# timghill/GladsGP

Hardware: NVIDIA B200
Metric: mcmc_steps_per_s (higher is better)
Workload: dtype f64

## Files before the change

gladsgp_b200/csrc/ggp_mcmc.cu:

```cuda
#include "ggp_chol.cuh"
#include "../../include/gladsgp_b200.h"

namespace ggp {

enum { PRIOR_UNIFORM = 0, PRIOR_GAMMA = 1, PRIOR_BETA = 2, PRIOR_NORMAL = 3 };
enum { PROP_UNIFORM = 0, PROP_BETARHO = 1, PROP_PROPMH = 2 };

__device__ inline double elem_log_prior(int kind, double a, double b, double x)
{
    switch (kind) {
        case PRIOR_GAMMA: return (a - 1.0) * log(x) - b * x;
        case PRIOR_BETA: {
            double rho = exp(-x / 4.0);
            if (rho > 0.999) rho = 0.999;
            return (a - 1.0) * log(rho) + (b - 1.0) * log(1.0 - rho);
        }
        case PRIOR_NORMAL: {
            double z = (x - a) / b;
            return -0.5 * (z * z);
        }
        default: return 0.0;
    }
}

struct Plan {
    double* cand;
    double* lacorr;
    double* logu;
    int* valid;
};

__device__ inline void plan_chain(const ggp_mcmc_args& a, const Plan& pl, int t, int c)
{
    const int P = a.d * a.pu + 2 * a.pu + 1;
    const double* th = a.theta + (size_t)c * P;
    const double* step = a.step + (size_t)t * a.step_stride_t + (size_t)c * a.step_stride_c;
    long long pos = a.upos ? a.upos[c] : 0;
    const double* us = a.uniforms ? a.uniforms + (size_t)c * a.n_uniform : nullptr;
    for (int s = 0; s < P; ++s) {
        const size_t o = (size_t)c * P + s;
        double cand, lac = 0.0, lu = 0.0;
        int valid;
        if (a.fixed[s] == 2) {
            pl.cand[o] = th[s]; pl.lacorr[o] = 0.0; pl.logu[o] = 0.0; pl.valid[o] = 0;
            continue;
        }
        if (a.replay) {
            const size_t ro = ((size_t)t * a.n_chains + c) * P + s;
            cand = a.r_cand[ro];
            lac = a.r_logacorr[ro];
            lu = a.r_logu[ro];
            valid = a.r_valid[ro] && !a.fixed[s];
        } else {
            const double x = th[s];
            const double st = step[s];
            const double u = us[pos++];
            double acorr = 1.0;
            int kind = a.prop_kind[s];
            if (kind == PROP_PROPMH && !a.do_propMH) kind = PROP_UNIFORM;
            if (kind == PROP_UNIFORM) {
                cand = __dadd_rn(x, __dmul_rn(st, __dadd_rn(-0.5, u)));
            } else if (kind == PROP_BETARHO) {
                const double rho = __dadd_rn(exp(-x / 4.0), __dmul_rn(st, __dadd_rn(-0.5, u)));
                cand = (rho <= 0.0) ? INFINITY : -4.0 * log(rho);
            } else {
                const double w = fmax(1.0, x / 3.0);
                cand = __dadd_rn(x, __dmul_rn(w, __dadd_rn(-1.0, __dmul_rn(2.0, u))));
                const double w1 = fmax(1.0, cand / 3.0);
                acorr = (x > cand + w1) ? 0.0 : w / w1;
            }
            valid = !a.fixed[s] && (acorr > 0.0) && (cand >= a.lo[s]) && (cand <= a.hi[s]);
            if (valid) {
                lu = log(us[pos++]);
                lac = log(acorr);
            }
        }
        pl.cand[o] = cand;
        pl.lacorr[o] = lac;
        pl.logu[o] = lu;
        pl.valid[o] = valid;
    }
    if (a.upos) a.upos[c] = pos;
}

__global__ void plan_kernel(ggp_mcmc_args a, Plan pl, int t)
{
    const int c = blockIdx.x * blockDim.x + threadIdx.x;
    if (c < a.n_chains) plan_chain(a, pl, t, c);
}

__device__ __forceinline__ const double* chain_w(const ggp_mcmc_args& a, int c, int j)
{
    return a.W + ((size_t)(a.per_chain_data ? c : 0) * a.pu + j) * a.m;
}
__device__ __forceinline__ double chain_lamsim(const ggp_mcmc_args& a, int c, int j)
{
    return a.lamsim[(size_t)(a.per_chain_data ? c : 0) * a.pu + j];
}
__device__ __forceinline__ size_t chain_prior_off(const ggp_mcmc_args& a, int c)
{
    return a.per_chain_data ? (size_t)c * ((size_t)a.d * a.pu + 2 * a.pu + 1) : 0;
}

__device__ inline void gather_block_params(const ggp_mcmc_args& a, const double* th, int c, int j, int site, double cand,
                                           double* beta_sm, double& lamz, double& diag_add)
{
    const int d = a.d, pu = a.pu, P = d * pu + 2 * pu + 1;
    if (threadIdx.x < d) {
        const int s = j * d + threadIdx.x;
        beta_sm[threadIdx.x] = (s == site) ? cand : th[s];
    }
    const int sz = d * pu + j, ss = d * pu + pu + j, so = P - 1;
    lamz = (sz == site) ? cand : th[sz];
    const double lamws = (ss == site) ? cand : th[ss];
    const double lamwos = (so == site) ? cand : th[so];
    diag_add = 1.0 / (chain_lamsim(a, c, j) * lamwos) + 1.0 / lamws;
}

#ifndef GGP_EVAL_INLINE
#define GGP_EVAL_INLINE 0
#endif
#if GGP_EVAL_INLINE
#define GGP_EVAL_ATTR __forceinline__
#else
#define GGP_EVAL_ATTR __noinline__
#endif
static __device__ GGP_EVAL_ATTR double eval_la_call(unsigned char* smem_raw, const double* __restrict__ X, int m, int Mp, int d,
                                                    const double* beta, double lamz, double diag_add,
                                                    const double* __restrict__ w, double* __restrict__ Lp, int rot)
{
    LaSmem sm = carve_la_smem(smem_raw, Mp, d);
    return eval_block_loglik_la(sm, X, m, Mp, d, beta, lamz, diag_add, w, Lp, nullptr, nullptr, rot);
}

template <bool CL, bool LA, int RA>
static __device__ __forceinline__ double eval_dispatch(unsigned char* smem_raw, const double* __restrict__ X, int m, int Mp, int d,
                                                       const double* beta, double lamz, double diag_add,
                                                       const double* __restrict__ w, double* __restrict__ Lp, int rot = 0)
{
    if constexpr (LA) {
        return eval_la_call(smem_raw, X, m, Mp, d, beta, lamz, diag_add, w, Lp, rot);
    } else {
        EvalSmem sm = carve_eval_smem(smem_raw, Mp, d);
        return eval_block_loglik<CL, RA>(sm, X, m, Mp, d, beta, lamz, diag_add, w, Lp, nullptr, nullptr);
    }
}

__device__ inline void finalize_chain(const ggp_mcmc_args& a, const Plan& pl, const double* __restrict__ sig_cand, int t, int c)
{
    const int d = a.d, pu = a.pu, P = d * pu + 2 * pu + 1;
    double* th = a.theta + (size_t)c * P;
    double* sig = a.sigwl + (size_t)c * pu;
    const int s = P - 1;
    const size_t o = (size_t)c * P + s;
    int acc = 0;
    if (pl.valid[o]) {
        double sn = 0.0, so = 0.0;
        for (int j = 0; j < pu; ++j) {
            sn += sig_cand[(size_t)c * pu + j];
            so += sig[j];
        }
        const double cand = pl.cand[o];
        const size_t po = chain_prior_off(a, c) + s;
        const double dprior = elem_log_prior(a.prior_kind[s], a.prior_a[po], a.prior_b[po], cand) -
                              elem_log_prior(a.prior_kind[s], a.prior_a[po], a.prior_b[po], th[s]);
        acc = pl.logu[o] < ((sn - so) + dprior) + pl.lacorr[o];
        if (acc) {
            th[s] = cand;
            for (int j = 0; j < pu; ++j) sig[j] = sig_cand[(size_t)c * pu + j];
        }
    }
    if (a.accepted) a.accepted[((size_t)t * a.n_chains + c) * P + s] = (unsigned char)acc;
    if (a.lp_draws) {
        double ll = 0.0;
        for (int j = 0; j < pu; ++j) ll += sig[j];
        double lpr = 0.0;
        const int bounds[5] = {0, d * pu, d * pu + pu, d * pu + 2 * pu, P};
        for (int blk = 0; blk < 4; ++blk) {
            if (a.fixed[bounds[blk]] == 2) continue;
            double sblk = 0.0;
            for (int e = bounds[blk]; e < bounds[blk + 1]; ++e)
                sblk += elem_log_prior(a.prior_kind[e], a.prior_a[chain_prior_off(a, c) + e], a.prior_b[chain_prior_off(a, c) + e], th[e]);
            lpr += sblk;
        }
        a.lp_draws[(size_t)t * a.n_chains + c] = ll + lpr;
    }
    if (a.draws) {
        double* dr = a.draws + ((size_t)t * a.n_chains + c) * P;
        for (int e = 0; e < P; ++e) dr[e] = th[e];
    }
}

template <bool CL, bool LA = false, int RA = GGP_RA>
__global__ void __launch_bounds__(NT, CL ? GGP_CL_CTAS_PER_SM : GGP_CTAS_PER_SM)
sweep_kernel(ggp_mcmc_args a, Plan pl, double* __restrict__ Lws, long long l_stride, double* __restrict__ sig_cand,
             unsigned* __restrict__ arrive, int t)
{
    extern __shared__ __align__(16) unsigned char smem_raw[];
    const int Mp = round_up32(a.m);
    __shared__ double beta_sm[64];
    const int j = a.pc_begin + (CL ? blockIdx.x / cluster_nctarank() : blockIdx.x), c = blockIdx.y;
    const bool lead = (threadIdx.x == 0) && (!CL || cluster_ctarank() == 0);
    const int d = a.d, pu = a.pu, P = d * pu + 2 * pu + 1;
    double* th = a.theta + (size_t)c * P;
    double* sig = a.sigwl + (size_t)c * pu;
    double* Lp = Lws + ((size_t)c * pu + j) * l_stride;
    const double* wj = chain_w(a, c, j);
    unsigned char* accd = a.accepted ? a.accepted + ((size_t)t * a.n_chains + c) * P : nullptr;
    const int rot = LA ? cta_role_rotation() : 0;
    const bool shard = a.pc_count > 0;
    double* xrow = shard ? a.xchg + ((size_t)j * a.n_chains + c) * (2 * d + 6) : nullptr;
    if (shard && lead) {
        xrow[d + 3] = sig[j];
        for (int e = 0; e < d + 2; ++e) xrow[d + 4 + e] = 0.0;
    }

    for (int sl = 0; sl < d + 3; ++sl) {
        const bool wos = (sl == d + 2);
        const int s = wos ? P - 1 : ((sl < d) ? j * d + sl : (sl == d ? d * pu + j : d * pu + pu + j));
        const size_t o = (size_t)c * P + s;
        const int valid = pl.valid[o];
        if (!valid) {
            if (lead && accd && !wos) accd[s] = 0;
            continue;
        }
        const double cand = pl.cand[o];
        double lamz, diag_add;
        __syncthreads();
        gather_block_params(a, th, c, j, s, cand, beta_sm, lamz, diag_add);
        __syncthreads();
        const double ll_new = eval_dispatch<CL, LA, RA>(smem_raw, a.X, a.m, Mp, d, beta_sm, lamz, diag_add, wj, Lp, rot);
        if (lead) {
            if (a.eval_count) atomicAdd(a.eval_count + (wos ? 1 : 0), 1ULL);
            if (wos) {
                sig_cand[(size_t)c * pu + j] = ll_new;
            } else {
                const double ll_old = sig[j];
                const double xold = th[s];
                const size_t po = chain_prior_off(a, c) + s;
                const double dprior = elem_log_prior(a.prior_kind[s], a.prior_a[po], a.prior_b[po], cand) -
                                      elem_log_prior(a.prior_kind[s], a.prior_a[po], a.prior_b[po], xold);
                const bool acc = pl.logu[o] < ((ll_new - ll_old) + dprior) + pl.lacorr[o];
                if (acc) {
                    th[s] = cand;
                    sig[j] = ll_new;
                }
                if (accd) accd[s] = acc ? 1 : 0;
                if (shard) xrow[d + 4 + sl] = acc ? 1.0 : 0.0;
            }
        }
        if (CL) cluster_sync_all();
        else __syncthreads();
    }
    if (lead && shard) {
        for (int e = 0; e < d; ++e) xrow[e] = th[j * d + e];
        xrow[d] = th[d * pu + j];
        xrow[d + 1] = th[d * pu + pu + j];
        xrow[d + 2] = sig[j];
        if (pl.valid[(size_t)c * P + (P - 1)]) xrow[d + 3] = sig_cand[(size_t)c * pu + j];
    } else if (lead) {
        __threadfence();
        const unsigned prev = atomicAdd(&arrive[c], 1u);
        if (prev == (unsigned)pu - 1u) {
            arrive[c] = 0u;
            __threadfence();
            finalize_chain(a, pl, sig_cand, t, c);
            if (t + 1 < a.n_steps) plan_chain(a, pl, t + 1, c);
        }
    }
}

constexpr int SPEC_LANES = 3;
constexpr int SPEC_MAXEV = 72;

__device__ __forceinline__ unsigned ld_acquire_u32(const unsigned* p)
{
    unsigned v;
    asm volatile("ld.acquire.gpu.global.u32 %0, [%1];" : "=r"(v) : "l"(p) : "memory");
    return v;
}

__device__ inline void gather_spec(const ggp_mcmc_args& a, const double* st, double lamwos_cur, int c, int j,
                                   int ea, double ca, int eb, double cb, double* beta_sm, double& lamz, double& diag_add)
{
    const int d = a.d;
    if (threadIdx.x < d) {
        const int e = threadIdx.x;
        beta_sm[e] = (e == ea) ? ca : ((e == eb) ? cb : st[e]);
    }
    lamz = (ea == d) ? ca : ((eb == d) ? cb : st[d]);
    const double lamws = (ea == d + 1) ? ca : ((eb == d + 1) ? cb : st[d + 1]);
    const double lamwos = (ea == d + 2) ? ca : ((eb == d + 2) ? cb : lamwos_cur);
    diag_add = 1.0 / (chain_lamsim(a, c, j) * lamwos) + 1.0 / lamws;
}

struct SpecWs {
    double* res;
    unsigned* cnt;
    double* state;
    double* Lws;
};

template <int RA>
__global__ void __launch_bounds__(NT, GGP_CL_CTAS_PER_SM)
sweep_spec_kernel(ggp_mcmc_args a, Plan pl, SpecWs sw, long long l_stride, double* __restrict__ sig_cand,
                  unsigned* __restrict__ arrive, int t, unsigned round_base)
{
    extern __shared__ __align__(16) unsigned char smem_raw[];
    __shared__ double beta_sm[64];
    __shared__ int ev_sm[SPEC_MAXEV];
    __shared__ int nev_sm;
    const int Mp = round_up32(a.m);
    const int G = (int)cluster_nctarank();
    const int cl = blockIdx.x / G;
    const int jl = cl / SPEC_LANES, lane_id = cl - jl * SPEC_LANES, c = blockIdx.y;
    const int j = a.pc_begin + jl;
    const bool lead = (threadIdx.x == 0) && (cluster_ctarank() == 0);
    const bool shard = a.pc_count > 0;
    const int d = a.d, pu = a.pu, P = d * pu + 2 * pu + 1;
    const int E = d + 3;
    double* th = a.theta + (size_t)c * P;
    double* st = sw.state + (((size_t)c * pu + j) * SPEC_LANES + lane_id) * (d + 3);
    double* Lp = sw.Lws + (((size_t)c * pu + j) * SPEC_LANES + lane_id) * l_stride;
    double* res = sw.res + ((size_t)c * pu + j) * 8;
    unsigned* cnt = sw.cnt + (size_t)c * pu + j;
    const double* wj = chain_w(a, c, j);
    unsigned char* accd = a.accepted ? a.accepted + ((size_t)t * a.n_chains + c) * P : nullptr;
    const double lamwos_cur = th[P - 1];
    double* xrow = shard ? a.xchg + ((size_t)j * a.n_chains + c) * (2 * d + 6) : nullptr;
    if (shard && lead && lane_id == 0) {
        xrow[d + 3] = a.sigwl[(size_t)c * pu + j];
        for (int e = 0; e < d + 2; ++e) xrow[d + 4 + e] = 0.0;
    }
    auto site_of = [&](int e) { return e < d ? j * d + e : (e == d ? d * pu + j : (e == d + 1 ? d * pu + pu + j : P - 1)); };

    if (threadIdx.x == 0) {
        int n = 0;
        for (int e = 0; e < E; ++e) {
            if (pl.valid[(size_t)c * P + site_of(e)]) ev_sm[n++] = e;
            else if (lead && accd && lane_id == 0 && e < d + 2) accd[site_of(e)] = 0;
        }
        nev_sm = n;
        if (cluster_ctarank() == 0) {
            for (int e = 0; e < d; ++e) st[e] = th[j * d + e];
            st[d] = th[d * pu + j];
            st[d + 1] = th[d * pu + pu + j];
            st[d + 2] = a.sigwl[(size_t)c * pu + j];
        }
    }
    cluster_sync_all();
    const int nev = nev_sm;
    const int nrounds = (nev + 1) >> 1;

    for (int r = 0; r < nrounds; ++r) {
        const int e0 = ev_sm[2 * r];
        const int e1 = (2 * r + 1 < nev) ? ev_sm[2 * r + 1] : -1;
        const size_t o0 = (size_t)c * P + site_of(e0);
        const size_t o1 = (e1 >= 0) ? (size_t)c * P + site_of(e1) : 0;
        const double c0 = pl.cand[o0];
        const double c1 = (e1 >= 0) ? pl.cand[o1] : 0.0;
        const bool work = (lane_id == 0) || (e1 >= 0);
        double ll = 0.0;
        if (work) {
            double lamz, diag_add;
            __syncthreads();
            if (lane_id == 0) gather_spec(a, st, lamwos_cur, c, j, e0, c0, -1, 0.0, beta_sm, lamz, diag_add);
            else if (lane_id == 1) gather_spec(a, st, lamwos_cur, c, j, e0, c0, e1, c1, beta_sm, lamz, diag_add);
            else gather_spec(a, st, lamwos_cur, c, j, e1, c1, -1, 0.0, beta_sm, lamz, diag_add);
            __syncthreads();
            ll = eval_dispatch<true, false, RA>(smem_raw, a.X, a.m, Mp, d, beta_sm, lamz, diag_add, wj, Lp, 0);
        }
        if (lead) {
            if (work && a.eval_count) atomicAdd(a.eval_count, 1ULL);
            double* slot = res + (r & 1) * 4;
            slot[lane_id] = ll;
            __threadfence();
            atomicAdd(cnt, 1u);
            const unsigned target = (round_base + (unsigned)r + 1u) * SPEC_LANES;
            const long long t0 = clock64();
            bool ok = true;
            while ((int)(ld_acquire_u32(cnt) - target) < 0) {
                if (clock64() - t0 > (1LL << 33)) { ok = false; break; }
            }
            const double l0 = __ldcg(slot + 0), l1a = __ldcg(slot + 1), l1r = __ldcg(slot + 2);
            if (!ok && a.lp_draws) a.lp_draws[(size_t)t * a.n_chains + c] = NAN;
            bool acc0 = false;
            if (e0 == d + 2) {
                if (lane_id == 0) sig_cand[(size_t)c * pu + j] = l0;
            } else {
                const int s0 = site_of(e0);
                const size_t po = chain_prior_off(a, c) + s0;
                const double dprior = elem_log_prior(a.prior_kind[s0], a.prior_a[po], a.prior_b[po], c0) -
                                      elem_log_prior(a.prior_kind[s0], a.prior_a[po], a.prior_b[po], st[e0]);
                acc0 = pl.logu[o0] < ((l0 - st[d + 2]) + dprior) + pl.lacorr[o0];
                if (acc0) { st[e0] = c0; st[d + 2] = l0; }
                if (accd && lane_id == 0) accd[s0] = acc0 ? 1 : 0;
                if (shard && lane_id == 0) xrow[d + 4 + e0] = acc0 ? 1.0 : 0.0;
            }
            if (e1 >= 0) {
                const double l1 = acc0 ? l1a : l1r;
                if (e1 == d + 2) {
                    if (lane_id == 0) sig_cand[(size_t)c * pu + j] = l1;
                } else {
                    const int s1 = site_of(e1);
                    const size_t po = chain_prior_off(a, c) + s1;
                    const double dprior = elem_log_prior(a.prior_kind[s1], a.prior_a[po], a.prior_b[po], c1) -
                                          elem_log_prior(a.prior_kind[s1], a.prior_a[po], a.prior_b[po], st[e1]);
                    const bool acc1 = pl.logu[o1] < ((l1 - st[d + 2]) + dprior) + pl.lacorr[o1];
                    if (acc1) { st[e1] = c1; st[d + 2] = l1; }
                    if (accd && lane_id == 0) accd[s1] = acc1 ? 1 : 0;
                    if (shard && lane_id == 0) xrow[d + 4 + e1] = acc1 ? 1.0 : 0.0;
                }
            }
        }
        cluster_sync_all();
    }
    if (lead) {
        const int rcap = (E + 1) >> 1;
        if (nrounds < rcap) atomicAdd(cnt, (unsigned)(rcap - nrounds));
        if (lane_id == 0 && shard) {
            for (int e = 0; e < d + 3; ++e) xrow[e] = st[e];
            if (pl.valid[(size_t)c * P + (P - 1)]) xrow[d + 3] = sig_cand[(size_t)c * pu + j];
        } else if (lane_id == 0) {
            for (int e = 0; e < d; ++e) th[j * d + e] = st[e];
            th[d * pu + j] = st[d];
            th[d * pu + pu + j] = st[d + 1];
            a.sigwl[(size_t)c * pu + j] = st[d + 2];
            __threadfence();
            const unsigned prev = atomicAdd(&arrive[c], 1u);
            if (prev == (unsigned)pu - 1u) {
                arrive[c] = 0u;
                __threadfence();
                finalize_chain(a, pl, sig_cand, t, c);
                if (t + 1 < a.n_steps) plan_chain(a, pl, t + 1, c);
            }
        }
    }
}

template <bool CL, bool LA = false, int RA = GGP_RA>
__global__ void __launch_bounds__(NT, CL ? GGP_CL_CTAS_PER_SM : GGP_CTAS_PER_SM)
eval_all_kernel(ggp_mcmc_args a, Plan pl, double* __restrict__ Lws, long long l_stride,
                double* __restrict__ sig_cand, int mode)
{
    extern __shared__ __align__(16) unsigned char smem_raw[];
    const int Mp = round_up32(a.m);
    __shared__ double beta_sm[64];
    const int j = CL ? blockIdx.x / cluster_nctarank() : blockIdx.x, c = blockIdx.y;
    const int d = a.d, pu = a.pu, P = d * pu + 2 * pu + 1;
    const double* th = a.theta + (size_t)c * P;
    double* Lp = Lws + ((size_t)c * pu + j) * l_stride;
    int site = -1;
    double cand = 0.0;
    if (mode == 1) {
        const size_t o = (size_t)c * P + (P - 1);
        if (!pl.valid[o]) return;
        site = P - 1;
        cand = pl.cand[o];
    }
    double lamz, diag_add;
    const int rot = LA ? cta_role_rotation() : 0;
    gather_block_params(a, th, c, j, site, cand, beta_sm, lamz, diag_add);
    __syncthreads();
    const double ll = eval_dispatch<CL, LA, RA>(smem_raw, a.X, a.m, Mp, d, beta_sm, lamz, diag_add, chain_w(a, c, j), Lp, rot);
    if (threadIdx.x == 0 && (!CL || cluster_ctarank() == 0)) {
        if (mode == 0) a.sigwl[(size_t)c * pu + j] = ll;
        else sig_cand[(size_t)c * pu + j] = ll;
        if (a.eval_count) atomicAdd(a.eval_count + 1, 1ULL);
    }
}

__global__ void close_kernel(ggp_mcmc_args a, Plan pl, double* __restrict__ sig_cand, int t, int plan_next)
{
    const int c = blockIdx.x * blockDim.x + threadIdx.x;
    if (c >= a.n_chains) return;
    const int d = a.d, pu = a.pu, P = d * pu + 2 * pu + 1;
    double* th = a.theta + (size_t)c * P;
    double* sig = a.sigwl + (size_t)c * pu;
    unsigned char* accd = a.accepted ? a.accepted + ((size_t)t * a.n_chains + c) * P : nullptr;
    for (int j = 0; j < pu; ++j) {
        const double* row = a.xchg + ((size_t)j * a.n_chains + c) * (2 * d + 6);
        for (int e = 0; e < d; ++e) th[j * d + e] = row[e];
        th[d * pu + j] = row[d];
        th[d * pu + pu + j] = row[d + 1];
        sig[j] = row[d + 2];
        sig_cand[(size_t)c * pu + j] = row[d + 3];
        if (accd) {
            for (int e = 0; e < d; ++e) accd[j * d + e] = (unsigned char)(row[d + 4 + e] != 0.0);
            accd[d * pu + j] = (unsigned char)(row[d + 4 + d] != 0.0);
            accd[d * pu + pu + j] = (unsigned char)(row[d + 4 + d + 1] != 0.0);
        }
    }
    finalize_chain(a, pl, sig_cand, t, c);
    if (plan_next) plan_chain(a, pl, t + 1, c);
}

static size_t align256(size_t x) { return (x + 255) & ~(size_t)255; }

static int spec_cluster_size(int pu, int n_chains, int Mp, int d)
{
    if (const char* e = getenv("GGP_SPEC")) { if (atoi(e) == 0) return 0; }
    if (d + 3 > SPEC_MAXEV) return 0;
    const int g_plain = choose_cluster((long long)pu * n_chains, Mp);
    if (g_plain <= 1) return 0;
    const int g_spec = choose_cluster((long long)SPEC_LANES * pu * n_chains, Mp);
    return (g_spec >= 2 && 2 * g_spec > g_plain) ? g_spec : 0;
}

struct McmcWs {
    double* Lws; Plan pl; double* sig_cand; unsigned* arrive; SpecWs spec;
};
long long workspace_bytes_impl(int m, int d, int pu, int n_chains, bool with_spec);

static McmcWs carve_ws(const ggp_mcmc_args& a)
{
    const int Mp = round_up32(a.m);
    const size_t P = (size_t)a.d * a.pu + 2 * a.pu + 1;
    McmcWs w;
    unsigned char* p = reinterpret_cast<unsigned char*>(a.workspace);
    w.Lws = reinterpret_cast<double*>(p);
    p += align256((size_t)a.n_chains * a.pu * packed_doubles(Mp) * sizeof(double));
    w.pl.cand = reinterpret_cast<double*>(p);   p += align256((size_t)a.n_chains * P * sizeof(double));
    w.pl.lacorr = reinterpret_cast<double*>(p); p += align256((size_t)a.n_chains * P * sizeof(double));
    w.pl.logu = reinterpret_cast<double*>(p);   p += align256((size_t)a.n_chains * P * sizeof(double));
    w.pl.valid = reinterpret_cast<int*>(p);     p += align256((size_t)a.n_chains * P * sizeof(int));
    w.sig_cand = reinterpret_cast<double*>(p);  p += align256((size_t)a.n_chains * a.pu * sizeof(double));
    w.arrive = reinterpret_cast<unsigned*>(p);  p += align256((size_t)a.n_chains * sizeof(unsigned));
    w.spec.res = nullptr; w.spec.cnt = nullptr; w.spec.state = nullptr; w.spec.Lws = nullptr;
    if (spec_cluster_size(1, a.n_chains, Mp, a.d) > 0 &&
        (long long)a.workspace_bytes >= workspace_bytes_impl(a.m, a.d, a.pu, a.n_chains, true)) {
        w.spec.res = reinterpret_cast<double*>(p);   p += align256((size_t)a.n_chains * a.pu * 8 * sizeof(double));
        w.spec.cnt = reinterpret_cast<unsigned*>(p); p += align256((size_t)a.n_chains * a.pu * sizeof(unsigned));
        w.spec.state = reinterpret_cast<double*>(p); p += align256((size_t)a.n_chains * a.pu * SPEC_LANES * (a.d + 3) * sizeof(double));
        w.spec.Lws = reinterpret_cast<double*>(p);
    }
    return w;
}

}

using namespace ggp;

extern "C" {

int ggp_sizeof_mcmc_args(void) { return (int)sizeof(ggp_mcmc_args); }

}

long long ggp::workspace_bytes_impl(int m, int d, int pu, int n_chains, bool with_spec)
{
    if (m <= 0 || d <= 0 || pu <= 0 || n_chains <= 0) return -1;
    const int Mp = round_up32(m);
    const size_t P = (size_t)d * pu + 2 * pu + 1;
    size_t b = 0;
    b += align256((size_t)n_chains * pu * packed_doubles(Mp) * sizeof(double));
    b += 3 * align256((size_t)n_chains * P * sizeof(double));
    b += align256((size_t)n_chains * P * sizeof(int));
    b += align256((size_t)n_chains * pu * sizeof(double));
    b += align256((size_t)n_chains * sizeof(unsigned));
    if (with_spec) {
        b += align256((size_t)n_chains * pu * 8 * sizeof(double));
        b += align256((size_t)n_chains * pu * sizeof(unsigned));
        b += align256((size_t)n_chains * pu * SPEC_LANES * (d + 3) * sizeof(double));
        b += align256((size_t)n_chains * pu * SPEC_LANES * packed_doubles(Mp) * sizeof(double));
    }
    return (long long)b;
}

extern "C" {

long long ggp_mcmc_workspace_bytes(int m, int d, int pu, int n_chains)
{
// ... 205 lines not shown
```

gladsgp_b200/ops.py:

```python
import ctypes as C
import numpy as np

from . import _lib
from ._lib import ptr, stream_ptr, check, McmcArgs


def _f64(t, torch, dev):
    return torch.as_tensor(np.ascontiguousarray(t, dtype=np.float64) if not torch.is_tensor(t) else t,
                           dtype=torch.float64, device=dev).contiguous()


def cov_build(X, beta, lamz, diag_add):
    torch = _lib.require_cuda()
    lib = _lib.load()
    dev = 'cuda'
    X = _f64(X, torch, dev); beta = _f64(beta, torch, dev).reshape(-1, X.shape[1])
    lamz = _f64(lamz, torch, dev).reshape(-1); diag_add = _f64(diag_add, torch, dev).reshape(-1)
    B, (m, d) = beta.shape[0], X.shape
    out = torch.empty((B, m, m), dtype=torch.float64, device=dev)
    check(lib.ggp_cov_build_f64(ptr(X), m, d, ptr(beta), ptr(lamz), ptr(diag_add), B, ptr(out), stream_ptr()),
          'ggp_cov_build_f64')
    return out


def cross_cov(X, Xp, beta, lamz):
    torch = _lib.require_cuda()
    lib = _lib.load()
    dev = 'cuda'
    X = _f64(X, torch, dev); Xp = _f64(Xp, torch, dev)
    beta = _f64(beta, torch, dev).reshape(-1, X.shape[1]); lamz = _f64(lamz, torch, dev).reshape(-1)
    B, (m, d), n = beta.shape[0], X.shape, Xp.shape[0]
    out = torch.empty((B, m, n), dtype=torch.float64, device=dev)
    check(lib.ggp_cross_cov_f64(ptr(X), m, ptr(Xp), n, d, ptr(beta), ptr(lamz), B, ptr(out), stream_ptr()),
          'ggp_cross_cov_f64')
    return out


def loglik_batched(X, W, beta, lamz, diag_add, want_factor=False, want_u=False, factor_ws=None):
    torch = _lib.require_cuda()
    lib = _lib.load()
    dev = 'cuda'
    X = _f64(X, torch, dev); W = _f64(W, torch, dev)
    beta = _f64(beta, torch, dev).reshape(-1, X.shape[1])
    lamz = _f64(lamz, torch, dev).reshape(-1); diag_add = _f64(diag_add, torch, dev).reshape(-1)
    B, (m, d) = beta.shape[0], X.shape
    assert W.shape == (B, m)
    fd = lib.ggp_factor_doubles(m)
    Mp = lib.ggp_padded_m(m)
    if factor_ws is None:
        factor_ws = torch.empty((B, fd), dtype=torch.float64, device=dev)
    u = torch.empty((B, Mp), dtype=torch.float64, device=dev) if want_u else None
    ll = torch.empty(B, dtype=torch.float64, device=dev)
    info = torch.empty(B, dtype=torch.int32, device=dev)
    check(lib.ggp_loglik_batched_f64(ptr(X), m, d, ptr(W), W.stride(0), ptr(beta), ptr(lamz), ptr(diag_add), B,
                                     ptr(factor_ws), ptr(u), ptr(ll), ptr(info), stream_ptr()),
          'ggp_loglik_batched_f64')
    out = dict(loglik=ll, info=info)
    if want_factor:
        out['factor'] = factor_ws
    if want_u:
        out['u'] = u
    return out


def factor_unpack(factor_ws, m):
    torch = _lib.require_cuda()
    lib = _lib.load()
    B = factor_ws.shape[0]
    out = torch.empty((B, m, m), dtype=torch.float64, device=factor_ws.device)
    check(lib.ggp_factor_unpack_f64(ptr(factor_ws), m, B, ptr(out), stream_ptr()), 'ggp_factor_unpack_f64')
    return out


PRIOR_KIND = {'Uniform': 0, 'Gamma': 1, 'Beta': 2, 'Normal': 3}
PROP_KIND = {'Uniform': 0, 'BetaRho': 1, 'PropMH': 2}


class McmcEngine:

    def __init__(self, X, W, lamsim, tables, n_chains=1, per_chain=False):
        torch = _lib.require_cuda()
        self.torch = torch
        self.lib = _lib.load()
        dev = 'cuda'
        self.per_chain = bool(per_chain)
        self.X = _f64(X, torch, dev); self.W = _f64(W, torch, dev); self.lamsim = _f64(lamsim, torch, dev)
        self.m, self.d = self.X.shape
        self.n_chains = int(n_chains)
        if self.per_chain:
            if self.W.dim() != 3 or self.W.shape[0] != self.n_chains or self.W.shape[2] != self.m:
                raise ValueError('per_chain: W must be (n_chains, pu, m)')
            self.pu = self.W.shape[1]
            if tuple(self.lamsim.shape) != (self.n_chains, self.pu):
                raise ValueError('per_chain: lamsim must be (n_chains, pu)')
        else:
            self.pu = self.W.shape[0]
        self.P = self.d * self.pu + 2 * self.pu + 1
        self.set_tables(tables)
        nb = self.lib.ggp_mcmc_workspace_bytes(self.m, self.d, self.pu, self.n_chains)
        self.ws = torch.empty(nb, dtype=torch.uint8, device=dev)
        self._pin = {}
        self._h2d_done = None
        self.theta = torch.zeros((self.n_chains, self.P), dtype=torch.float64, device=dev)
        self.sigwl = torch.zeros((self.n_chains, self.pu), dtype=torch.float64, device=dev)
        self.upos = torch.zeros(self.n_chains, dtype=torch.int64, device=dev)
        self.launches_per_step = 1

    def set_tables(self, tb):
        torch, dev = self.torch, 'cuda'
        P = self.P
        self.t_prior_kind = torch.as_tensor(np.asarray(tb['prior_kind'], dtype=np.int32).reshape(P), device=dev)
        pshape = (self.n_chains, P) if self.per_chain else (P,)
        self.t_prior_a = _f64(np.asarray(tb['prior_a']).reshape(pshape), torch, dev)
        self.t_prior_b = _f64(np.asarray(tb['prior_b']).reshape(pshape), torch, dev)
        self.t_lo = _f64(np.asarray(tb['lo']).reshape(P), torch, dev)
        self.t_hi = _f64(np.asarray(tb['hi']).reshape(P), torch, dev)
        self.t_prop_kind = torch.as_tensor(np.asarray(tb['prop_kind'], dtype=np.int32).reshape(P), device=dev)
        self.t_fixed = torch.as_tensor(np.asarray(tb['fixed'], dtype=np.uint8).reshape(P), device=dev)

    def set_state(self, theta):
        th = _f64(np.asarray(theta, dtype=np.float64).reshape(-1, self.P), self.torch, 'cuda')
        if th.shape[0] == 1 and self.n_chains > 1:
            th = th.expand(self.n_chains, self.P)
        self.theta.copy_(th)

    def _build_args(self, n_steps, step, uniforms, replay, do_propMH, init_sigwl, record, record_accept):
        torch, dev = self.torch, 'cuda'
        a = McmcArgs()
        a.m, a.d, a.pu, a.n_chains, a.n_steps = self.m, self.d, self.pu, self.n_chains, int(n_steps)
        a.do_propMH, a.init_sigwl = int(bool(do_propMH)), int(bool(init_sigwl))
        a.per_chain_data = int(self.per_chain)
        keep = []
        step = _f64(step, torch, dev); keep.append(step)
        if step.dim() == 1:
            a.step_stride_t, a.step_stride_c = 0, 0
        elif step.shape[0] == n_steps and step.dim() == 2:
            a.step_stride_t, a.step_stride_c = self.P, 0
        elif step.dim() == 3 and step.shape[0] == 1:
            a.step_stride_t, a.step_stride_c = 0, self.P
        elif step.dim() == 3:
            a.step_stride_t, a.step_stride_c = self.n_chains * self.P, self.P
        else:
            raise ValueError('step must be (P,), (n_steps,P) or (n_steps,n_chains,P)')
        a.X, a.W, a.lamsim = self.X.data_ptr(), self.W.data_ptr(), self.lamsim.data_ptr()
        a.prior_kind, a.prior_a, a.prior_b = self.t_prior_kind.data_ptr(), self.t_prior_a.data_ptr(), self.t_prior_b.data_ptr()
        a.lo, a.hi = self.t_lo.data_ptr(), self.t_hi.data_ptr()
        a.prop_kind, a.fixed = self.t_prop_kind.data_ptr(), self.t_fixed.data_ptr()
        a.step = step.data_ptr()
        a.theta, a.sigwl = self.theta.data_ptr(), self.sigwl.data_ptr()
        if replay is not None:
            a.replay = 1
            sh = (n_steps, self.n_chains, self.P)
            rc = _f64(np.asarray(replay['cand']).reshape(sh), torch, dev)
            ra = _f64(np.asarray(replay['logacorr']).reshape(sh), torch, dev)
            ru = _f64(np.asarray(replay['logu']).reshape(sh), torch, dev)
            rv = torch.as_tensor(np.asarray(replay['valid'], dtype=np.uint8).reshape(sh), device=dev)
            keep += [rc, ra, ru, rv]
            a.r_cand, a.r_logacorr, a.r_logu, a.r_valid = rc.data_ptr(), ra.data_ptr(), ru.data_ptr(), rv.data_ptr()
        else:
            a.replay = 0
            if not torch.is_tensor(uniforms):
                uniforms = torch.as_tensor(np.ascontiguousarray(uniforms, dtype=np.float64))
            uniforms = uniforms.reshape(self.n_chains, -1)
            if uniforms.device.type != 'cuda':
                if self._h2d_done is not None:
                    self._h2d_done.synchronize()
                stage = self._pinned('uniforms', uniforms.numel(), torch.float64)
                stage.copy_(uniforms.reshape(-1))
                uniforms = stage.to(dev, non_blocking=True).reshape(self.n_chains, -1)
                self._h2d_done = torch.cuda.Event()
                self._h2d_done.record()
            keep.append(uniforms)
            a.uniforms, a.n_uniform = uniforms.data_ptr(), uniforms.shape[1]
            self.upos.zero_()
            a.upos = self.upos.data_ptr()
        draws = lp = acc = None
        if record:
            draws = torch.empty((n_steps, self.n_chains, self.P), dtype=torch.float64, device=dev)
            lp = torch.empty((n_steps, self.n_chains), dtype=torch.float64, device=dev)
            a.draws, a.lp_draws = draws.data_ptr(), lp.data_ptr()
        if record_accept:
            acc = torch.empty((n_steps, self.n_chains, self.P), dtype=torch.uint8, device=dev)
            a.accepted = acc.data_ptr()
        a.workspace, a.workspace_bytes = self.ws.data_ptr(), self.ws.numel()
        return a, keep, draws, lp, acc

    def run(self, n_steps, step, uniforms=None, replay=None, do_propMH=True, init_sigwl=True,
            record=True, record_accept=False, time_kernels=False):
        torch, dev = self.torch, 'cuda'
        a, keep, draws, lp, acc = self._build_args(n_steps, step, uniforms, replay, do_propMH, init_sigwl, record, record_accept)
        kms = (C.c_double * 2)(0.0, 0.0)
        cnt = None
        if time_kernels:
            a.kernel_ms = C.cast(kms, C.c_void_p)
            cnt = torch.zeros(2, dtype=torch.int64, device=dev)
            a.eval_count = cnt.data_ptr()
        check(self.lib.ggp_mcmc_run_f64(C.byref(a), stream_ptr()), 'ggp_mcmc_run_f64')
        self._keep = keep
        return dict(draws=draws, lp=lp, accepted=acc, consumed=self.upos,
                    kernel_ms=(kms[0], kms[1]) if time_kernels else None,
                    eval_count=cnt.cpu().numpy() if cnt is not None else None)

    def run_by_pc(self, n_steps, step, uniforms=None, replay=None, do_propMH=True, init_sigwl=True,
                  record=True, record_accept=False, shards=None, gather=None):
        torch, dev = self.torch, 'cuda'
        a, keep, draws, lp, acc = self._build_args(n_steps, step, uniforms, replay, do_propMH, init_sigwl, record, record_accept)
        if shards is None:
            shards = [(0, self.pu)]
        rows = self.pu if gather is None else gather.padded_pcs
        xchg = torch.zeros((rows, self.n_chains, 2 * self.d + 6), dtype=torch.float64, device=dev)
        a.xchg = xchg.data_ptr()
        total_steps = int(n_steps)
        a.n_steps = 1
        sp = stream_ptr
        a.pc_begin, a.pc_count = 0, 0
        check(self.lib.ggp_mcmc_plan_f64(C.byref(a), 0, sp()), 'ggp_mcmc_plan_f64')
        for t in range(total_steps):
            a.step_index = t
            first = True
            for (b, cnt) in shards:
                if cnt <= 0:
                    continue
                a.pc_begin, a.pc_count = int(b), int(cnt)
                a.init_sigwl = int(bool(init_sigwl) and t == 0 and first)
                first = False
                check(self.lib.ggp_mcmc_run_f64(C.byref(a), sp()), 'ggp_mcmc_run_f64 (PC shard)')
            if gather is not None:
                gather(xchg)
            a.pc_begin, a.pc_count = 0, 0
            check(self.lib.ggp_mcmc_close_f64(C.byref(a), t, int(t + 1 < total_steps), sp()), 'ggp_mcmc_close_f64')
        self._keep = keep + [xchg]
        return dict(draws=draws, lp=lp, accepted=acc, consumed=self.upos, kernel_ms=None, eval_count=None)

    def _pinned(self, name, numel, dtype):
        buf = self._pin.get(name)
        if buf is None or buf.numel() < numel or buf.dtype != dtype:
            buf = self.torch.empty(max(int(numel), 1), dtype=dtype).pin_memory()
            self._pin[name] = buf
        return buf[:numel]

    def to_host(self, t, name):
        stage = self._pinned(name, t.numel(), t.dtype)
        stage.copy_(t.reshape(-1), non_blocking=True)
        self.torch.cuda.current_stream().synchronize()
        return stage.numpy().reshape(tuple(t.shape)).copy()


class Predictor:

    def __init__(self, X, W, beta, lamz, diag_add, s11_diag):
        torch = _lib.require_cuda()
        self.torch, self.lib = torch, _lib.load()
        dev = 'cuda'
        self.X = _f64(X, torch, dev)
        self.m, self.d = self.X.shape
        self.beta = _f64(beta, torch, dev).reshape(-1, self.d)
        self.B = self.beta.shape[0]
        self.lamz = _f64(lamz, torch, dev).reshape(-1)
        self.s11 = _f64(s11_diag, torch, dev).reshape(-1)
        self.W = _f64(W, torch, dev).reshape(self.B, self.m)
        out = loglik_batched(self.X, self.W, self.beta, self.lamz, diag_add, want_factor=True, want_u=True)
        self.factor, self.u, self.loglik, self.info = out['factor'], out['u'], out['loglik'], out['info']
        self.Mp = self.u.shape[1]
        self._ws = None
        self._xws = None

    def predict(self, Xp, want_V=False):
        torch, lib, dev = self.torch, self.lib, 'cuda'
        Xp = _f64(Xp, torch, dev)
        n = Xp.shape[0]
        need = lib.ggp_predict_workspace_bytes(self.m, n, self.B)
# ... 362 lines not shown
```

Before: 3627.

## Skip likelihood evaluation for beta sites on constant input columns

When an input column of X is constant, its beta parameter cannot change the GP covariance, so the likelihood is unchanged. Such sites are marked neutral on the host, and the plan kernel decides accept or reject from the prior ratio alone. The per-site and speculative loops then apply the accepted candidate without running a Cholesky evaluation. This helps only when X has constant columns, and it adds a new three-state site encoding that both kernels must handle consistently.

```diff
diff --git a/gladsgp_b200/csrc/ggp_mcmc.cu b/gladsgp_b200/csrc/ggp_mcmc.cu
--- a/gladsgp_b200/csrc/ggp_mcmc.cu
+++ b/gladsgp_b200/csrc/ggp_mcmc.cu
@@ -23,12 +23,22 @@
     }
 }
 
+enum { SITE_REJECT = 0,
+       SITE_EVAL = 1,
+       SITE_ACCEPT = 2 };
+enum { FIXED_NEUTRAL = 3 };
+
 struct Plan {
     double* cand;
     double* lacorr;
     double* logu;
     int* valid;
 };
+
+__device__ __forceinline__ size_t chain_prior_off(const ggp_mcmc_args& a, int c)
+{
+    return a.per_chain_data ? (size_t)c * ((size_t)a.d * a.pu + 2 * a.pu + 1) : 0;
+}
 
 __device__ inline void plan_chain(const ggp_mcmc_args& a, const Plan& pl, int t, int c)
 {
@@ -42,15 +52,17 @@
         double cand, lac = 0.0, lu = 0.0;
         int valid;
         if (a.fixed[s] == 2) {
-            pl.cand[o] = th[s]; pl.lacorr[o] = 0.0; pl.logu[o] = 0.0; pl.valid[o] = 0;
+            pl.cand[o] = th[s]; pl.lacorr[o] = 0.0; pl.logu[o] = 0.0; pl.valid[o] = SITE_REJECT;
             continue;
         }
+        const bool neutral = a.fixed[s] == FIXED_NEUTRAL && s < a.d * a.pu;
+        const bool sampled = a.fixed[s] == 0 || neutral;
         if (a.replay) {
             const size_t ro = ((size_t)t * a.n_chains + c) * P + s;
             cand = a.r_cand[ro];
             lac = a.r_logacorr[ro];
             lu = a.r_logu[ro];
-            valid = a.r_valid[ro] && !a.fixed[s];
+            valid = a.r_valid[ro] && sampled;
         } else {
             const double x = th[s];
             const double st = step[s];
@@ -69,11 +81,17 @@
                 const double w1 = fmax(1.0, cand / 3.0);
                 acorr = (x > cand + w1) ? 0.0 : w / w1;
             }
-            valid = !a.fixed[s] && (acorr > 0.0) && (cand >= a.lo[s]) && (cand <= a.hi[s]);
+            valid = sampled && (acorr > 0.0) && (cand >= a.lo[s]) && (cand <= a.hi[s]);
             if (valid) {
                 lu = log(us[pos++]);
                 lac = log(acorr);
             }
+        }
+        if (valid && neutral && isfinite(cand)) {
+            const size_t po = chain_prior_off(a, c) + s;
+            const double dprior = elem_log_prior(a.prior_kind[s], a.prior_a[po], a.prior_b[po], cand) -
+                                  elem_log_prior(a.prior_kind[s], a.prior_a[po], a.prior_b[po], th[s]);
+            valid = (lu < dprior + lac) ? SITE_ACCEPT : SITE_REJECT;
         }
         pl.cand[o] = cand;
         pl.lacorr[o] = lac;
@@ -97,11 +115,6 @@
 {
     return a.lamsim[(size_t)(a.per_chain_data ? c : 0) * a.pu + j];
 }
-__device__ __forceinline__ size_t chain_prior_off(const ggp_mcmc_args& a, int c)
-{
-    return a.per_chain_data ? (size_t)c * ((size_t)a.d * a.pu + 2 * a.pu + 1) : 0;
-}
-
 __device__ inline void gather_block_params(const ggp_mcmc_args& a, const double* th, int c, int j, int site, double cand,
                                            double* beta_sm, double& lamz, double& diag_add)
 {
@@ -220,8 +233,14 @@
         const int s = wos ? P - 1 : ((sl < d) ? j * d + sl : (sl == d ? d * pu + j : d * pu + pu + j));
         const size_t o = (size_t)c * P + s;
         const int valid = pl.valid[o];
-        if (!valid) {
-            if (lead && accd && !wos) accd[s] = 0;
+        if (valid != SITE_EVAL) {
+            const bool acc = valid == SITE_ACCEPT;
+            if (lead && !wos) {
+                if (acc) th[s] = pl.cand[o];
+                if (accd) accd[s] = acc ? 1 : 0;
+                if (shard) xrow[d + 4 + sl] = acc ? 1.0 : 0.0;
+            }
+            if (CL && acc) cluster_sync_all();
             continue;
         }
         const double cand = pl.cand[o];
@@ -281,12 +300,13 @@
 }
 
 __device__ inline void gather_spec(const ggp_mcmc_args& a, const double* st, double lamwos_cur, int c, int j,
-                                   int ea, double ca, int eb, double cb, double* beta_sm, double& lamz, double& diag_add)
+                                   int ea, double ca, int eb, double cb, unsigned long long nacc, const double* ncand, int lim,
+                                   double* beta_sm, double& lamz, double& diag_add)
 {
     const int d = a.d;
     if (threadIdx.x < d) {
         const int e = threadIdx.x;
-        beta_sm[e] = (e == ea) ? ca : ((e == eb) ? cb : st[e]);
+        beta_sm[e] = (e == ea) ? ca : ((e == eb) ? cb : ((e < lim && ((nacc >> e) & 1ULL)) ? ncand[e] : st[e]));
     }
     lamz = (ea == d) ? ca : ((eb == d) ? cb : st[d]);
     const double lamws = (ea == d + 1) ? ca : ((eb == d + 1) ? cb : st[d + 1]);
@@ -310,6 +330,7 @@
     __shared__ double beta_sm[64];
     __shared__ int ev_sm[SPEC_MAXEV];
     __shared__ int nev_sm;
+    __shared__ unsigned long long nacc_sm;
     const int Mp = round_up32(a.m);
     const int G = (int)cluster_nctarank();
     const int cl = blockIdx.x / G;
@@ -333,14 +354,25 @@
         for (int e = 0; e < d + 2; ++e) xrow[d + 4 + e] = 0.0;
     }
     auto site_of = [&](int e) { return e < d ? j * d + e : (e == d ? d * pu + j : (e == d + 1 ? d * pu + pu + j : P - 1)); };
+    const double* ncand = pl.cand + (size_t)c * P + (size_t)j * d;
 
     if (threadIdx.x == 0) {
         int n = 0;
+        unsigned long long nacc = 0ULL;
         for (int e = 0; e < E; ++e) {
-            if (pl.valid[(size_t)c * P + site_of(e)]) ev_sm[n++] = e;
-            else if (lead && accd && lane_id == 0 && e < d + 2) accd[site_of(e)] = 0;
+            const int v = pl.valid[(size_t)c * P + site_of(e)];
+            if (v == SITE_EVAL) {
+                ev_sm[n++] = e;
+                continue;
+            }
+            if (v == SITE_ACCEPT) nacc |= 1ULL << e;
+            if (lead && lane_id == 0 && e < d + 2) {
+                if (accd) accd[site_of(e)] = (v == SITE_ACCEPT) ? 1 : 0;
+                if (shard) xrow[d + 4 + e] = (v == SITE_ACCEPT) ? 1.0 : 0.0;
+            }
         }
         nev_sm = n;
+        nacc_sm = nacc;
         if (cluster_ctarank() == 0) {
             for (int e = 0; e < d; ++e) st[e] = th[j * d + e];
             st[d] = th[d * pu + j];
@@ -350,6 +382,7 @@
     }
     cluster_sync_all();
     const int nev = nev_sm;
+    const unsigned long long nacc = nacc_sm;
     const int nrounds = (nev + 1) >> 1;
 
     for (int r = 0; r < nrounds; ++r) {
@@ -364,9 +397,9 @@
         if (work) {
             double lamz, diag_add;
             __syncthreads();
-            if (lane_id == 0) gather_spec(a, st, lamwos_cur, c, j, e0, c0, -1, 0.0, beta_sm, lamz, diag_add);
-            else if (lane_id == 1) gather_spec(a, st, lamwos_cur, c, j, e0, c0, e1, c1, beta_sm, lamz, diag_add);
-            else gather_spec(a, st, lamwos_cur, c, j, e1, c1, -1, 0.0, beta_sm, lamz, diag_add);
+            if (lane_id == 0) gather_spec(a, st, lamwos_cur, c, j, e0, c0, -1, 0.0, nacc, ncand, e0, beta_sm, lamz, diag_add);
+            else if (lane_id == 1) gather_spec(a, st, lamwos_cur, c, j, e0, c0, e1, c1, nacc, ncand, e1, beta_sm, lamz, diag_add);
+            else gather_spec(a, st, lamwos_cur, c, j, e1, c1, -1, 0.0, nacc, ncand, e1, beta_sm, lamz, diag_add);
             __syncthreads();
             ll = eval_dispatch<true, false, RA>(smem_raw, a.X, a.m, Mp, d, beta_sm, lamz, diag_add, wj, Lp, 0);
         }
@@ -418,6 +451,9 @@
     if (lead) {
         const int rcap = (E + 1) >> 1;
         if (nrounds < rcap) atomicAdd(cnt, (unsigned)(rcap - nrounds));
+        if (lane_id == 0)
+            for (int e = 0; e < d; ++e)
+                if ((nacc >> e) & 1ULL) st[e] = ncand[e];
         if (lane_id == 0 && shard) {
             for (int e = 0; e < d + 3; ++e) xrow[e] = st[e];
             if (pl.valid[(size_t)c * P + (P - 1)]) xrow[d + 3] = sig_cand[(size_t)c * pu + j];
diff --git a/gladsgp_b200/ops.py b/gladsgp_b200/ops.py
--- a/gladsgp_b200/ops.py
+++ b/gladsgp_b200/ops.py
@@ -74,6 +74,17 @@
 
 PRIOR_KIND = {'Uniform': 0, 'Gamma': 1, 'Beta': 2, 'Normal': 3}
 PROP_KIND = {'Uniform': 0, 'BetaRho': 1, 'PropMH': 2}
+FIXED_NEUTRAL = 3
+
+
+def mark_neutral_sites(X, fixed, pu):
+    X = np.asarray(X, dtype=np.float64)
+    d = X.shape[1]
+    const = np.all(X == X[:1], axis=0) & np.all(np.isfinite(X), axis=0)
+    fx = np.array(fixed, dtype=np.uint8).reshape(-1)
+    beta = fx[:d * pu].reshape(pu, d)
+    beta[(beta == 0) & const[None, :]] = FIXED_NEUTRAL
+    return fx
 
 
 class McmcEngine:
@@ -96,6 +107,7 @@
         else:
             self.pu = self.W.shape[0]
         self.P = self.d * self.pu + 2 * self.pu + 1
+        self.X_host = self.X.cpu().numpy()
         self.set_tables(tables)
         nb = self.lib.ggp_mcmc_workspace_bytes(self.m, self.d, self.pu, self.n_chains)
         self.ws = torch.empty(nb, dtype=torch.uint8, device=dev)
@@ -116,7 +128,8 @@
         self.t_lo = _f64(np.asarray(tb['lo']).reshape(P), torch, dev)
         self.t_hi = _f64(np.asarray(tb['hi']).reshape(P), torch, dev)
         self.t_prop_kind = torch.as_tensor(np.asarray(tb['prop_kind'], dtype=np.int32).reshape(P), device=dev)
-        self.t_fixed = torch.as_tensor(np.asarray(tb['fixed'], dtype=np.uint8).reshape(P), device=dev)
+        fixed = mark_neutral_sites(self.X_host, np.asarray(tb['fixed'], dtype=np.uint8).reshape(P), self.pu)
+        self.t_fixed = torch.as_tensor(fixed, device=dev)
 
     def set_state(self, theta):
         th = _f64(np.asarray(theta, dtype=np.float64).reshape(-1, self.P), self.torch, 'cuda')
```

Measured after the change: 3846, median of 6. +6.0%, better.
